# ashvardanian/StringZilla

Hardware: AMD Instinct MI355X
Metric: DP cell-updates/s (GCUPS) on 1M-pair Levenshtein batch (higher is better)
Workload: dtype u32 bit-vectors (u64 results)

## Files before the change

stringzilla_amd/csrc/hip/lev_myers.hip:

```cpp
#include "myers_core.hpp"

#define SZS_PAIR_RULE_FN __host__ __device__ static inline
#include "pair_rule.h"

#include <cstdlib>

namespace szs_hip {

#ifndef SZS_MYERS_PACK_QUERIES
#define SZS_MYERS_PACK_QUERIES 1
#endif
#ifndef SZS_MYERS_PAIR_RULES
#define SZS_MYERS_PAIR_RULES 1
#endif

#ifndef SZS_MYERS_SHORT_TEXT_DWORDS
#define SZS_MYERS_SHORT_TEXT_DWORDS 2
#endif


__device__ __forceinline__ u32 bits_in_word(u32 from, u32 to, int w) {
    u32 const low = from > 32u * w ? from : 32u * w, high = to < 32u * w + 32u ? to : 32u * w + 32u;
    if (low >= high) return 0u;
    return (high - low == 32u ? ~0u : (1u << (high - low)) - 1u) << (low - 32u * w);
}

template <int words_, int text_dwords_, bool runes_, bool paired_ = false>
__device__ __forceinline__ void myers_workgroup(u32 *peq, u32 *keys, szs_string_ref_t const query,
                                                szs_string_ref_t const *__restrict__ candidates, u32 candidates_count,
                                                u32 candidate_block, u64 *__restrict__ results, u64 results_row_stride,
                                                int symmetric, szs_ref_guard_t const &guard, u32 alphabet = 0,
                                                u32 *claimed_rows = nullptr, u32 blocks_here = 1, szs_string_ref_t const second = {}) {
    static_assert(!paired_ || !runes_, "query pairs are a byte-kernel shape");
    constexpr int rows = runes_ ? rune_slots_k : byte_rows_k;
    using layout = peq_layout<words_, rows>;
    if (guard.enabled && (!ref_is_current(guard, 0, query) || (paired_ && !ref_is_current(guard, 0, second)))) {
        if (threadIdx.x == 0) *guard.stale = guard.sequence;
        return;
    }
    u32 const first_length = query.length, second_length = paired_ ? second.length : 0u;
    u32 const query_length = paired_ ? first_length + second_length : first_length;
    u32 const used_rows = paired_ ? query_length + 2u : query_length;
    u32 const pad = 32u * words_ - used_rows;
    u32 const second_row = pad + first_length + 2u;

    for (int i = threadIdx.x; i < layout::total_dwords; i += 256) peq[i] = 0;
    if constexpr (runes_) {
        if (alphabet) {
            for (u32 i = threadIdx.x; i <= alphabet; i += 256) keys[i] = 0;
            if (threadIdx.x == 0) *claimed_rows = 0;
        }
        else
            for (int i = threadIdx.x; i < rune_slots_k; i += 256) keys[i] = rune_slot_empty_k;
    }
    __syncthreads();
    if (runes_ && alphabet) {
        u32 const *pattern = reinterpret_cast<u32 const *>(query.address);
        for (u32 i = threadIdx.x; i < query_length; i += 256) {
            u32 const id = pattern[i];
            if (atomicCAS(&keys[id], 0u, ~0u) == 0u) keys[id] = atomicAdd(claimed_rows, 1u) + 1;
        }
        __syncthreads();
        for (u32 i = threadIdx.x; i < query_length; i += 256) {
            u32 const position = pad + i;
            atomicOr(&peq[layout::dword_index((int)keys[pattern[i]], (int)(position >> 5))], 1u << (position & 31));
        }
    }
    else if constexpr (runes_) {
        u32 const *pattern = reinterpret_cast<u32 const *>(query.address);
        for (u32 i = threadIdx.x; i < query_length; i += 256) {
            u32 const rune = pattern[i];
            u32 slot = rune_slot_hash(rune);
            for (;;) {
                u32 const previous = atomicCAS(&keys[slot], rune_slot_empty_k, rune);
                if (previous == rune_slot_empty_k || previous == rune) break;
                slot = (slot + 1) & (rune_slots_k - 1);
            }
            u32 const position = pad + i;
            atomicOr(&peq[layout::dword_index((int)slot, (int)(position >> 5))], 1u << (position & 31));
        }
    }
    else {
        u8 const *pattern = reinterpret_cast<u8 const *>(query.address);
        for (u32 i = threadIdx.x; i < first_length; i += 256) {
            u32 const position = pad + i;
            atomicOr(&peq[layout::dword_index(pattern[i], (int)(position >> 5))], 1u << (position & 31));
        }
        if constexpr (paired_) {
            u8 const *above = reinterpret_cast<u8 const *>(second.address);
            for (u32 i = threadIdx.x; i < second_length; i += 256) {
                u32 const position = second_row + i;
                atomicOr(&peq[layout::dword_index(above[i], (int)(position >> 5))], 1u << (position & 31));
            }
        }
    }
    __syncthreads();
    pattern_pair_t<words_> boundary;
    if constexpr (paired_) {
#pragma unroll
        for (int w = 0; w < words_; ++w) {
            boundary.separators[w] = bits_in_word(second_row - 2u, second_row, w);
            boundary.tops[w] = first_length ? bits_in_word(second_row - 3u, second_row - 2u, w) : 0u;
        }
    }

#pragma unroll 1
    for (u32 block_step = 0; block_step < blocks_here; ++block_step) {
    u32 const candidate_slot = (candidate_block - block_step) * SZS_CANDIDATES_PER_WORKGROUP + threadIdx.x;
    bool live = candidate_slot < candidates_count;
    szs_string_ref_t candidate = {0, 0, 0};
    if (live) candidate = candidates[candidate_slot];
    if (live && guard.enabled && !ref_is_current(guard, 1, candidate)) {
        *guard.stale = guard.sequence;
        live = false;
    }
    if ((symmetric & SZS_LAYOUT_SYMMETRIC) && candidate.index > query.index) live = false;
    u32 const text_length = live ? candidate.length : 0;
    u32 const longest_in_wave = wave_max_u32(text_length);
    u32 const shortest_in_wave = ~wave_max_u32(live ? ~text_length : 0u);

    u32 vp[words_], vn[words_];
#pragma unroll
    for (int w = 0; w < words_; ++w) {
        vp[w] = bits_in_word(pad, 32u * words_, w) & ~(paired_ ? boundary.separators[w] : 0u);
        vn[w] = 0;
    }

    auto take = [&](u32 symbol) {
        u32 eq[words_];
        load_match_masks<words_, rows>(peq, !runes_ ? symbol : alphabet ? keys[symbol] : find_rune_slot(keys, symbol), eq);
        if constexpr (paired_) myers_column<words_>(vp, vn, eq, boundary);
        else myers_column<words_>(vp, vn, eq);
    };

    u32 column = 0;
    if constexpr (runes_) {
        u32 const *const runes = reinterpret_cast<u32 const *>(candidate.address);
        auto quad_at = [&](u32 index) -> uint4 {
            return index < text_length ? *reinterpret_cast<uint4 const *>(runes + index) : make_uint4(0, 0, 0, 0);
        };
        if (4 <= shortest_in_wave && longest_in_wave) {
            uint4 ahead = quad_at(0);
            for (; column + 4 <= shortest_in_wave; column += 4) {
                uint4 const now = ahead;
                ahead = quad_at(column + 4);
                take(now.x), take(now.y), take(now.z), take(now.w);
            }
        }
#pragma unroll 1
        for (; column < longest_in_wave; ++column)
            if (column < text_length) take(runes[column]);
    }
    else {
        u64 const safe_address = text_length ? candidate.address : first_length || !paired_ ? query.address : second.address;
        text_stream_t text(safe_address, text_length);
        if (!text_length) text.valid_dwords = query_length ? 1 : 0;
        u32 raw_low = text.raw(0);
        u32 dword = 0;
        constexpr u32 columns_per_iteration = 4 * text_dwords_;
#ifndef SZS_MYERS_CLAMPED_READS
#define SZS_MYERS_CLAMPED_READS(TEXT_DWORDS) ((TEXT_DWORDS) == 1)
#endif
        constexpr bool clamped_reads = SZS_MYERS_CLAMPED_READS(text_dwords_);
        if (columns_per_iteration <= shortest_in_wave && longest_in_wave && query_length) {
            u32 ahead[text_dwords_];
#pragma unroll
            for (int d = 0; d < text_dwords_; ++d) ahead[d] = clamped_reads ? text.raw_clamped(1 + d) : text.raw(1 + d);
            for (; column + columns_per_iteration <= shortest_in_wave;
                 column += columns_per_iteration, dword += text_dwords_) {
                u32 symbols[text_dwords_];
                symbols[0] = text.splice(raw_low, ahead[0]);
#pragma unroll
                for (int d = 1; d < text_dwords_; ++d) symbols[d] = text.splice(ahead[d - 1], ahead[d]);
                raw_low = ahead[text_dwords_ - 1];
#pragma unroll
                for (int d = 0; d < text_dwords_; ++d)
                    ahead[d] = clamped_reads ? text.raw_clamped(dword + text_dwords_ + 1 + d)
                                             : text.raw(dword + text_dwords_ + 1 + d);
#pragma unroll
                for (int step = 0; step < 4 * text_dwords_; ++step) take((symbols[step / 4] >> (8 * (step % 4))) & 0xFFu);
            }
        }
#ifndef SZS_MYERS_MID_LOOP
#define SZS_MYERS_MID_LOOP 0
#endif
        if constexpr (SZS_MYERS_MID_LOOP && text_dwords_ > 1) {
            if (column + 4 <= shortest_in_wave && longest_in_wave && query_length) {
                u32 ahead_one = text.raw(dword + 1);
#pragma unroll 1
                for (; column + 4 <= shortest_in_wave; column += 4, ++dword) {
                    u32 const symbols = text.splice(raw_low, ahead_one);
                    raw_low = ahead_one;
                    ahead_one = text.raw(dword + 2);
#pragma unroll
                    for (int step = 0; step < 4; ++step) take((symbols >> (8 * step)) & 0xFFu);
                }
            }
        }
        if (column < longest_in_wave) {
            u32 next = text.raw(dword + 1);
#pragma unroll 1
            for (; column < longest_in_wave; column += 4, ++dword) {
                u32 const after = text.raw(dword + 2);
                u32 const symbols = text.splice(raw_low, next);
                raw_low = next, next = after;
#pragma unroll
                for (int step = 0; step < 4; ++step)
                    if (column + step < text_length) take((symbols >> (8 * step)) & 0xFFu);
            }
        }
    }

    if (live && paired_) {
        u32 first = text_length, above = text_length;
#pragma unroll
        for (int w = 0; w < words_; ++w) {
            u32 const mine = bits_in_word(pad, pad + first_length, w), theirs = bits_in_word(second_row, 32u * words_, w);
            first += (u32)__builtin_popcount(vp[w] & mine) - (u32)__builtin_popcount(vn[w] & mine);
            above += (u32)__builtin_popcount(vp[w] & theirs) - (u32)__builtin_popcount(vn[w] & theirs);
        }
        bool const transposed = (symmetric & SZS_LAYOUT_TRANSPOSED) != 0;
        u64 const one = transposed ? candidate.index : query.index, two = transposed ? candidate.index : second.index;
        u64 const one_column = transposed ? query.index : candidate.index, two_column = transposed ? second.index : candidate.index;
        results[one * results_row_stride + one_column] = first;
        results[two * results_row_stride + two_column] = above;
    }
    else if (live) {
        u32 distance = text_length;
#pragma unroll
        for (int w = 0; w < words_; ++w) distance += (u32)__builtin_popcount(vp[w]) - (u32)__builtin_popcount(vn[w]);
        bool const transposed = (symmetric & SZS_LAYOUT_TRANSPOSED) != 0;
        u64 const row = transposed ? candidate.index : query.index, column = transposed ? query.index : candidate.index;
        results[row * results_row_stride + column] = distance;
        if ((symmetric & SZS_LAYOUT_SYMMETRIC) && candidate.index != query.index)
            results[column * results_row_stride + row] = distance;
    }
    }
}

#ifndef SZS_WORK_BLOCK_MAJOR
#define SZS_WORK_BLOCK_MAJOR 1
#endif
__device__ __forceinline__ void myers_work_item(u32 candidate_blocks, u32 &query_slot, u32 &candidate_block) {
#if SZS_WORK_BLOCK_MAJOR
    u32 const queries_count = gridDim.x / candidate_blocks;
    query_slot = blockIdx.x % queries_count;
    candidate_block = candidate_blocks - 1 - blockIdx.x / queries_count;
#else
    query_slot = blockIdx.x / candidate_blocks;
    candidate_block = candidate_blocks - 1 - blockIdx.x % candidate_blocks;
#endif
}

#ifndef SZS_MYERS_LONG_WAVES
#define SZS_MYERS_LONG_WAVES 2
#endif
template <int words_>
__global__ __launch_bounds__(256, SZS_MYERS_LONG_WAVES) void levenshtein_myers_long_kernel(szs_string_ref_t const *__restrict__ queries,
                                                                      szs_string_ref_t const *__restrict__ candidates,
                                                                      u32 candidates_count, u32 candidate_blocks,
                                                                      u64 *__restrict__ results, u64 results_row_stride,
                                                                      int symmetric, szs_ref_guard_t guard) {
    __shared__ __attribute__((aligned(16))) u32 peq[peq_layout<words_>::total_dwords];
    u32 query_slot, candidate_block;
    myers_work_item(candidate_blocks, query_slot, candidate_block);
    myers_workgroup<words_, 1, false>(peq, nullptr, queries[query_slot], candidates, candidates_count, candidate_block,
                                      results, results_row_stride, symmetric, guard);
}

__device__ __forceinline__ u64 fused_offset(void const *offsets, u32 wide, u64 index) {
    return wide ? static_cast<u64 const *>(offsets)[index] : (u64) static_cast<u32 const *>(offsets)[index];
}

__device__ __forceinline__ void fused_sort_side(szs_plan_side_t const &side, u32 is_query_side, u32 choose_rule, u32 sequence, u32 *ready,
                                                u32 second_ready, u32 withhold, szs_fused_side_report_t *report, u32 *histogram ,
                                                szs_string_ref_t *staged ) {
    constexpr u32 per_thread = SZS_FUSED_MOST_STRINGS / 256;
    u32 const tid = threadIdx.x, lane = tid & 63u, wave = tid >> 6, count = side.count;
    bool const one_pass = count <= SZS_FUSED_MOST_STRINGS;
    __shared__ u32 wave_bins[4], wave_longest[4], wave_status[4];
    __shared__ unsigned long long wave_symbols[4], wave_bands_systolic[4], wave_bands_chain[4], wave_squares[4];
    __shared__ u32 rule_words[256];

    u64 const began = wall_clock64();
    for (u32 bin = tid; bin < SZS_FUSED_BINS; bin += 256) histogram[bin] = 0;
    u64 from[per_thread], to[per_thread];
#pragma unroll
    for (u32 k = 0; k < per_thread; ++k) {
        u32 const i = tid + k * 256;
        from[k] = to[k] = 0;
        if (one_pass && i < count) from[k] = fused_offset(side.offsets, side.wide, i), to[k] = fused_offset(side.offsets, side.wide, (u64)i + 1);
    }
    __syncthreads();
    u32 bins[per_thread];
    u32 status = 0, longest = 0;
    u64 symbols = 0, bands_systolic = 0, bands_chain = 0, squares = 0;
    auto count_in = [&](u64 first, u64 last) -> u32 {
        if (last < first) return status |= SZS_PLAN_STATUS_DESCENDING, ~0u;
        if (last - first > 0xFFFFFFFFull) return status |= SZS_PLAN_STATUS_OVERFLOW, ~0u;
        u32 const length = (u32)(last - first);
        symbols += length, squares += (u64)length * length, longest = length > longest ? length : longest;
        bands_systolic += length ? (length + SZS_SYSTOLIC_BAND_ROWS - 1) / SZS_SYSTOLIC_BAND_ROWS : 1;
        bands_chain += length ? (length + SZS_MYERS_CHAIN_BAND_ROWS - 1) / SZS_MYERS_CHAIN_BAND_ROWS : 1;
        u32 const bin = length < SZS_FUSED_BINS - 1 ? length : SZS_FUSED_BINS - 1;
        atomicAdd(&histogram[bin], 1u);
        return bin;
    };
    if (one_pass) {
#pragma unroll
        for (u32 k = 0; k < per_thread; ++k) {
            bins[k] = ~0u;
            if (tid + k * 256 < count) bins[k] = count_in(from[k], to[k]);
        }
    }
    else {
#pragma unroll 1
        for (u32 first = 0; first < count; first += 1024) {
            u64 some_from[4], some_to[4];
#pragma unroll
            for (u32 k = 0; k < 4; ++k) {
                u32 const i = first + tid + k * 256;
                some_from[k] = some_to[k] = 0;
                if (i < count) some_from[k] = fused_offset(side.offsets, side.wide, i), some_to[k] = fused_offset(side.offsets, side.wide, (u64)i + 1);
            }
#pragma unroll
            for (u32 k = 0; k < 4; ++k)
                if (first + tid + k * 256 < count) (void)count_in(some_from[k], some_to[k]);
        }
    }
    if (tid == 0) report->ticks[0] = (u32)began, report->ticks[1] = (u32)(wall_clock64() - began);
#pragma unroll
    for (int offset = 32; offset >= 1; offset >>= 1) {
        status |= (u32)__shfl_xor((int)status, offset, 64);
        u32 const other = (u32)__shfl_xor((int)longest, offset, 64);
        longest = other > longest ? other : longest;
    }
    if (lane == 0) wave_status[wave] = status, wave_longest[wave] = longest;
    __syncthreads();
    u32 mine[4], sum = 0;
#pragma unroll
    for (u32 k = 0; k < 4; ++k) mine[k] = histogram[4 * tid + k], sum += mine[k];
    u32 inclusive = sum;
#pragma unroll
    for (int offset = 1; offset < 64; offset <<= 1) {
        u32 const other = (u32)__shfl_up((int)inclusive, offset, 64);
        if (lane >= (u32)offset) inclusive += other;
    }
    if (lane == 63) wave_bins[wave] = inclusive;
    __syncthreads();
    status = wave_status[0] | wave_status[1] | wave_status[2] | wave_status[3];
    longest = wave_longest[0];
#pragma unroll
    for (u32 w = 1; w < 4; ++w) longest = wave_longest[w] > longest ? wave_longest[w] : longest;
    u32 running = inclusive - sum;
    for (u32 w = 0; w < wave; ++w) running += wave_bins[w];
#pragma unroll
    for (u32 k = 0; k < 4; ++k) histogram[4 * tid + k] = running, running += mine[k];
    __syncthreads();
    if (tid == 0) report->ticks[2] = (u32)(wall_clock64() - began);
    u32 const blank = status || (is_query_side && longest > 32u * SZS_MYERS_SHORT_WORDS);
    if (one_pass) {
#pragma unroll
        for (u32 k = 0; k < per_thread; ++k) {
            u32 const i = tid + k * 256;
            if (i >= count) continue;
            szs_string_ref_t ref;
            ref.address = status ? side.base : side.base + from[k], ref.length = blank ? 0u : (u32)(to[k] - from[k]), ref.index = i;
            staged[status ? i : atomicAdd(&histogram[bins[k]], 1u)] = ref;
        }
        __syncthreads();
        for (u32 position = tid; position < count; position += 256) {
            szs_string_ref_t const ref = staged[position];
            side.ascending[position] = ref, side.descending[count - 1 - position] = ref;
        }
    }
    u32 const pair_slots = szs_pair_slots(count), pair_seconds = szs_pair_seconds(count);
    bool const choosing = choose_rule && one_pass && pair_seconds;
    if (choosing) {
        constexpr u32 strides = 256 / SZS_PAIR_RULE_CANDIDATES;
        u32 me = tid;
        asm volatile("" : "+v"(me));
        u32 const rule = szs_pair_rule_candidate(me % SZS_PAIR_RULE_CANDIDATES, pair_seconds);
        u32 words = 0;
        if (me < strides * SZS_PAIR_RULE_CANDIDATES) {
#pragma unroll 4
            for (u32 slot = me / SZS_PAIR_RULE_CANDIDATES; slot < pair_seconds; slot += strides)
                words += szs_pair_slot_words(staged[count - 1 - slot].length,
                                             staged[count - 1 - szs_pair_second_rank(rule, slot, pair_slots, pair_seconds)].length);
        }
        rule_words[me] = words;
    }
    if (!one_pass) {
#pragma unroll 1
        for (u32 first = 0; first < count; first += 1024) {
            u64 some_from[4], some_to[4];
#pragma unroll
            for (u32 k = 0; k < 4; ++k) {
                u32 const i = first + tid + k * 256;
                some_from[k] = some_to[k] = 0;
                if (i < count) some_from[k] = fused_offset(side.offsets, side.wide, i), some_to[k] = fused_offset(side.offsets, side.wide, (u64)i + 1);
            }
#pragma unroll
            for (u32 k = 0; k < 4; ++k) {
                u32 const i = first + tid + k * 256;
                if (i >= count) continue;
// ... 1351 lines not shown
```

stringzilla_amd/csrc/hip/myers_core.hpp:

```cpp
#pragma once
#include "device_common.hpp"

namespace szs_hip {

constexpr int byte_rows_k = 256;
constexpr int rune_slots_k = 512;
constexpr u32 rune_slot_empty_k = ~0u;

template <int words_, int rows_ = byte_rows_k>
struct peq_layout {
    static constexpr int chunk_words = words_ >= 3 ? 4 : words_;
    static constexpr int chunks = (words_ + chunk_words - 1) / chunk_words;
    static constexpr int total_dwords = chunks * rows_ * chunk_words;
    __device__ static constexpr int dword_index(int row, int w) {
        return ((w / chunk_words) * rows_ + row) * chunk_words + (w % chunk_words);
    }
};

__device__ __forceinline__ u32 rune_slot_hash(u32 rune) { return (rune * 2654435761u) >> 23; }
__device__ __forceinline__ u32 find_rune_slot(u32 const *keys, u32 rune) {
    u32 slot = rune_slot_hash(rune);
    for (;;) {
        u32 const key = keys[slot];
        if (key == rune || key == rune_slot_empty_k) return slot;
        slot = (slot + 1) & (rune_slots_k - 1);
    }
}

template <int words_, int rows_>
__device__ __forceinline__ void load_match_masks(u32 const *peq, u32 symbol, u32 (&eq)[words_]) {
    using layout = peq_layout<words_, rows_>;
    if constexpr (layout::chunk_words == 4) {
        uint4 const *rows = reinterpret_cast<uint4 const *>(peq);
#pragma unroll
        for (int chunk = 0; chunk < layout::chunks; ++chunk) {
            uint4 const row = rows[chunk * rows_ + symbol];
            if (chunk * 4 + 0 < words_) eq[chunk * 4 + 0] = row.x;
            if (chunk * 4 + 1 < words_) eq[chunk * 4 + 1] = row.y;
            if (chunk * 4 + 2 < words_) eq[chunk * 4 + 2] = row.z;
            if (chunk * 4 + 3 < words_) eq[chunk * 4 + 3] = row.w;
        }
    }
    else if constexpr (layout::chunk_words == 2) {
        uint2 const row = reinterpret_cast<uint2 const *>(peq)[symbol];
        eq[0] = row.x, eq[1] = row.y;
    }
    else { eq[0] = peq[symbol]; }
}

__device__ __forceinline__ bool ref_is_current(szs_ref_guard_t const &guard, int side, szs_string_ref_t const &ref) {
    if (ref.index >= guard.side[side].count) return false;
    u64 from, to;
    if (guard.side[side].wide) {
        u64 const *offsets = static_cast<u64 const *>(guard.side[side].offsets);
        from = offsets[ref.index], to = offsets[(u64)ref.index + 1];
    }
    else {
        u32 const *offsets = static_cast<u32 const *>(guard.side[side].offsets);
        from = offsets[ref.index], to = offsets[(u64)ref.index + 1];
    }
    return to >= from && to - from == ref.length && guard.side[side].base + from == ref.address;
}

struct single_pattern_t {
    __device__ static constexpr u32 separator(int) { return 0; }
    __device__ static constexpr u32 top(int) { return 0; }
};

template <int words_>
struct pattern_pair_t {
    u32 separators[words_], tops[words_];
    __device__ u32 separator(int w) const { return separators[w]; }
    __device__ u32 top(int w) const { return tops[w]; }
};

template <int words_, typename boundary_t = single_pattern_t, bool materialise_ = true>
__device__ __forceinline__ void myers_column(u32 (&vp)[words_], u32 (&vn)[words_], u32 const (&eq)[words_],
                                             boundary_t const &boundary = {}) {
    u32 carry = 0, hp_below = 0, hn_below = 0;
#pragma unroll
    for (int w = 0; w < words_; ++w) {
        u32 xv = eq[w] | vn[w];
        if constexpr (!std::is_same<boundary_t, single_pattern_t>::value)
            asm("v_bitop3_b32 %0, %1, %2, %3 bitop3:0xfe" : "=v"(xv) : "v"(eq[w]), "v"(vn[w]), "v"(boundary.separator(w)));
        u32 carry_out;
        u32 const sum = __builtin_addc(eq[w] & vp[w], vp[w], carry, &carry_out);
        carry = carry_out;
        u32 const d0 = (sum ^ vp[w]) | eq[w];
        u32 const hp = vn[w] | ~(d0 | vp[w]);
        u32 const hn = vp[w] & d0 & ~boundary.top(w);
        u32 const hp_shifted = w == 0 ? ((hp << 1) | 1u) : __builtin_amdgcn_alignbit(hp, hp_below, 31);
        u32 const hn_shifted = w == 0 ? (hn << 1) : __builtin_amdgcn_alignbit(hn, hn_below, 31);
        hp_below = hp, hn_below = hn;
        vp[w] = hn_shifted | ~(xv | hp_shifted);
        vn[w] = hp_shifted & xv & ~boundary.separator(w);
        if constexpr (materialise_ && words_ > 1) asm("" : "+v"(vp[w]), "+v"(vn[w]));
    }
}

template <int words_>
__device__ __forceinline__ u32 myers_infix_column(u32 (&vp)[words_], u32 (&vn)[words_], u32 const (&eq)[words_]) {
    u32 carry = 0, hp_below = 0, hn_below = 0;
#pragma unroll
    for (int w = 0; w < words_; ++w) {
        u32 const xv = eq[w] | vn[w];
        u32 carry_out;
        u32 const sum = __builtin_addc(eq[w] & vp[w], vp[w], carry, &carry_out);
        carry = carry_out;
        u32 const d0 = (sum ^ vp[w]) | eq[w];
        u32 const hp = vn[w] | ~(d0 | vp[w]);
        u32 const hn = vp[w] & d0;
        u32 const hp_shifted = w == 0 ? (hp << 1) : __builtin_amdgcn_alignbit(hp, hp_below, 31);
        u32 const hn_shifted = w == 0 ? (hn << 1) : __builtin_amdgcn_alignbit(hn, hn_below, 31);
        hp_below = hp, hn_below = hn;
        vp[w] = hn_shifted | ~(xv | hp_shifted);
        vn[w] = hp_shifted & xv;
        if constexpr (words_ > 1) asm("" : "+v"(vp[w]), "+v"(vn[w]));
    }
    return (hp_below >> 31) | ((hn_below >> 31) << 1);
}

template <int words_>
__device__ __forceinline__ u32 myers_prefix_column(u32 (&vp)[words_], u32 (&vn)[words_], u32 const (&eq)[words_]) {
    u32 carry = 0, hp_below = 0, hn_below = 0;
#pragma unroll
    for (int w = 0; w < words_; ++w) {
        u32 const xv = eq[w] | vn[w];
        u32 carry_out;
        u32 const sum = __builtin_addc(eq[w] & vp[w], vp[w], carry, &carry_out);
        carry = carry_out;
        u32 const d0 = (sum ^ vp[w]) | eq[w];
        u32 const hp = vn[w] | ~(d0 | vp[w]);
        u32 const hn = vp[w] & d0;
        u32 const hp_shifted = w == 0 ? ((hp << 1) | 1u) : __builtin_amdgcn_alignbit(hp, hp_below, 31);
        u32 const hn_shifted = w == 0 ? (hn << 1) : __builtin_amdgcn_alignbit(hn, hn_below, 31);
        hp_below = hp, hn_below = hn;
        vp[w] = hn_shifted | ~(xv | hp_shifted);
        vn[w] = hp_shifted & xv;
        if constexpr (words_ > 1) asm("" : "+v"(vp[w]), "+v"(vn[w]));
    }
    return (hp_below >> 31) | ((hn_below >> 31) << 1);
}

template <int words_>
__device__ __forceinline__ u32 myers_strip_column(u32 (&vp)[words_], u32 (&vn)[words_], u32 const (&eq)[words_], u32 hp_in,
                                                  u32 hn_in) {
    u32 carry = 0, hp_below = 0, hn_below = 0;
#pragma unroll
    for (int w = 0; w < words_; ++w) {
        u32 const xv = eq[w] | vn[w];
        u32 const eq_in = w == 0 ? (eq[w] | hn_in) : eq[w];
        u32 carry_out;
        u32 const sum = __builtin_addc(eq_in & vp[w], vp[w], carry, &carry_out);
        carry = carry_out;
        u32 const d0 = (sum ^ vp[w]) | eq_in;
        u32 const hp = vn[w] | ~(d0 | vp[w]);
        u32 const hn = vp[w] & d0;
        u32 const hp_shifted = w == 0 ? ((hp << 1) | hp_in) : __builtin_amdgcn_alignbit(hp, hp_below, 31);
        u32 const hn_shifted = w == 0 ? ((hn << 1) | hn_in) : __builtin_amdgcn_alignbit(hn, hn_below, 31);
        hp_below = hp, hn_below = hn;
        vp[w] = hn_shifted | ~(xv | hp_shifted);
        vn[w] = hp_shifted & xv;
    }
    return (hp_below >> 31) | ((hn_below >> 31) << 1);
}

}
```

stringzilla_amd/csrc/hip/myers_rerank.hip:

```cpp
#include "rerank_core.hpp"

namespace szs_hip {

template <int words_, int lanes_>
__device__ __forceinline__ void rerank_rows(u32 *table, listed_row_t const &row, szs_rerank_side_t const &candidates,
                                            u64 const *__restrict__ indices, u64 indices_stride, u64 k, u64 *__restrict__ scores,
                                            u64 scores_stride, u32 *flags, unsigned long long *counters) {
    u32 const sub = threadIdx.x % lanes_;
    u32 const pad = 32u * words_ - row.query_length;
    listed_table<words_, lanes_>(table, row, [](int) { return 0u; }, [&](u32 i) { return pad + i; });

    listed_counters_t counted;
#pragma unroll 1
    for (u64 first = 0; first < k; first += lanes_) {
        u64 const rank = first + sub;
        u64 const at = row.row * scores_stride + rank;
        u64 address = 0;
        u32 text_length = 0;
        bool const live = row.has_row && rank < k &&
                          listed_candidate(candidates, indices[row.row * indices_stride + rank], [&]() { scores[at] = 0; }, flags, address, text_length);

        u32 vp[words_], vn[words_];
#pragma unroll
        for (int w = 0; w < words_; ++w) vp[w] = rerank_bits_in_word(pad, 32u * words_, w), vn[w] = 0;
        listed_walk(
            text_stream_t(address, text_length), text_length, live,
            [&](u32 symbol, u32) {
                u32 eq[words_];
                load_match_masks<words_, byte_rows_k>(table, symbol, eq);
                myers_column<words_>(vp, vn, eq);
            },
            []() { return true; });

        if (live) {
            u32 distance = text_length;
#pragma unroll
            for (int w = 0; w < words_; ++w) distance += (u32)__builtin_popcount(vp[w]) - (u32)__builtin_popcount(vn[w]);
            scores[at] = distance;
            counted.add(row.query_length, text_length);
        }
    }
    counted.land(counters, true);
}

template <int lanes_>
__global__ __launch_bounds__(64) void levenshtein_rerank_kernel(szs_rerank_side_t const queries, szs_rerank_side_t const candidates,
                                                                u64 const first_query, u32 const *__restrict__ rows, u32 const rows_count,
                                                                u64 const *__restrict__ indices, u64 const indices_stride, u64 const k,
                                                                u64 *__restrict__ scores, u64 const scores_stride, u32 const table_dwords,
                                                                u32 *flags, unsigned long long *counters) {
    extern __shared__ __attribute__((aligned(16))) u32 rerank_tables[];
    listed_one_strip_rows<lanes_>(queries, first_query, rows, rows_count, rerank_tables, table_dwords, flags,
                                  [&](auto width, u32 *table, listed_row_t const &row) {
                                      rerank_rows<decltype(width)::value, lanes_>(table, row, candidates, indices, indices_stride, k, scores,
                                                                                  scores_stride, flags, counters);
                                  });
}

}

extern "C" unsigned szs_hip_rerank_lanes(uint64_t k) { return k <= 16 ? 16u : k <= 32 ? 32u : 64u; }

extern "C" int szs_hip_levenshtein_rerank(szs_rerank_side_t const *queries, szs_rerank_side_t const *candidates, uint64_t first_query,
                                          uint32_t const *rows, uint32_t rows_count, uint64_t const *indices, uint64_t indices_stride,
                                          uint64_t k, uint64_t *scores, uint64_t scores_stride, unsigned widest, uint32_t *flags,
                                          unsigned long long *counters, void *stream) {
    using namespace szs_hip;
    if (!rows_count || !k) return 0;
    if (widest < 1 || widest > SZS_MYERS_SHORT_WORDS || !queries || !candidates || !flags || !counters) return (int)hipErrorInvalidValue;
    listed_grid_t const grid = listed_one_strip_grid(k, rows_count, widest);
    return listed_launch(k, [&](auto lanes) {
        hipLaunchKernelGGL(levenshtein_rerank_kernel<decltype(lanes)::value>, dim3(grid.grid), dim3(wave_size_k), grid.lds,
                           static_cast<hipStream_t>(stream), *queries, *candidates, first_query, rows, rows_count, indices, indices_stride, k,
                           scores, scores_stride, grid.table_dwords, flags, counters);
    });
}
```

Before: 101,800.

## Rederive Myers column via shifted HN carry identity and bitop3 ternary ops

Rewrites the Myers bit-vector column update so the shifted horizontal-negative vector comes straight from the add's carry bits (sum ^ (eq|vp) ^ eq), removing the separate HN shift chain, and fuses most boolean steps into v_bitop3_b32 ternary instructions. For query pairs the boundary handling moves from a per-column 'top' mask to a 'lower' mask folded into the kept term, and the separator row is pre-seeded in the PEQ table at initialisation. This aims to cut VALU instructions and carried registers per DP column, in exchange for hand-derived truth tables that must stay exactly correct for paired boundaries. The rerank path opts out of spelled carries so the compiler can pick its own form.

Result: faster. 119,500, median of 6 (+17.4%).

```diff
diff --git a/stringzilla_amd/csrc/hip/lev_myers.hip b/stringzilla_amd/csrc/hip/lev_myers.hip
--- a/stringzilla_amd/csrc/hip/lev_myers.hip
+++ b/stringzilla_amd/csrc/hip/lev_myers.hip
@@ -44,7 +44,13 @@
     u32 const pad = 32u * words_ - used_rows;
     u32 const second_row = pad + first_length + 2u;
 
-    for (int i = threadIdx.x; i < layout::total_dwords; i += 256) peq[i] = 0;
+    if constexpr (paired_) {
+        u32 const s0_dword = (second_row - 2u) >> 5, s0_mask = 1u << ((second_row - 2u) & 31u);
+        for (int i = threadIdx.x; i < layout::total_dwords; i += 256)
+            peq[i] = (u32)(i / (rows * layout::chunk_words) * layout::chunk_words + i % layout::chunk_words) == s0_dword ? s0_mask : 0u;
+    }
+    else
+        for (int i = threadIdx.x; i < layout::total_dwords; i += 256) peq[i] = 0;
     if constexpr (runes_) {
         if (alphabet) {
             for (u32 i = threadIdx.x; i <= alphabet; i += 256) keys[i] = 0;
@@ -100,7 +106,7 @@
 #pragma unroll
         for (int w = 0; w < words_; ++w) {
             boundary.separators[w] = bits_in_word(second_row - 2u, second_row, w);
-            boundary.tops[w] = first_length ? bits_in_word(second_row - 3u, second_row - 2u, w) : 0u;
+            boundary.lower[w] = bits_in_word(second_row - 2u, second_row - 1u, w);
         }
     }
 
diff --git a/stringzilla_amd/csrc/hip/myers_core.hpp b/stringzilla_amd/csrc/hip/myers_core.hpp
--- a/stringzilla_amd/csrc/hip/myers_core.hpp
+++ b/stringzilla_amd/csrc/hip/myers_core.hpp
@@ -62,38 +62,47 @@
     return to >= from && to - from == ref.length && guard.side[side].base + from == ref.address;
 }
 
-struct single_pattern_t {
-    __device__ static constexpr u32 separator(int) { return 0; }
-    __device__ static constexpr u32 top(int) { return 0; }
-};
+struct single_pattern_t {};
 
 template <int words_>
 struct pattern_pair_t {
-    u32 separators[words_], tops[words_];
-    __device__ u32 separator(int w) const { return separators[w]; }
-    __device__ u32 top(int w) const { return tops[w]; }
+    u32 separators[words_], lower[words_];
 };
 
-template <int words_, typename boundary_t = single_pattern_t, bool materialise_ = true>
+template <int table_>
+__device__ __forceinline__ u32 bitop3(u32 a, u32 b, u32 c) {
+    u32 r;
+    asm("v_bitop3_b32 %0, %1, %2, %3 bitop3:%4" : "=v"(r) : "v"(a), "v"(b), "v"(c), "n"(table_));
+    return r;
+}
+
+template <int words_, typename boundary_t = single_pattern_t, bool materialise_ = true, bool spelled_carries_ = true>
 __device__ __forceinline__ void myers_column(u32 (&vp)[words_], u32 (&vn)[words_], u32 const (&eq)[words_],
                                              boundary_t const &boundary = {}) {
-    u32 carry = 0, hp_below = 0, hn_below = 0;
+    constexpr bool paired = !std::is_same<boundary_t, single_pattern_t>::value;
+    static_assert(spelled_carries_ || !paired, "a pair's HNs is not a function the compiler finds by itself");
+    u32 carry = 0, hp_below = 0;
 #pragma unroll
     for (int w = 0; w < words_; ++w) {
-        u32 xv = eq[w] | vn[w];
-        if constexpr (!std::is_same<boundary_t, single_pattern_t>::value)
-            asm("v_bitop3_b32 %0, %1, %2, %3 bitop3:0xfe" : "=v"(xv) : "v"(eq[w]), "v"(vn[w]), "v"(boundary.separator(w)));
+        u32 xv, kept, hn_shifted;
+        if constexpr (paired) {
+            xv = bitop3<0xfe>(eq[w], vn[w], boundary.separators[w]);
+            kept = bitop3<0x54>(eq[w], vp[w], boundary.lower[w]);
+        }
+        else
+            xv = eq[w] | vn[w], kept = eq[w] | vp[w];
         u32 carry_out;
         u32 const sum = __builtin_addc(eq[w] & vp[w], vp[w], carry, &carry_out);
         carry = carry_out;
-        u32 const d0 = (sum ^ vp[w]) | eq[w];
-        u32 const hp = vn[w] | ~(d0 | vp[w]);
-        u32 const hn = vp[w] & d0 & ~boundary.top(w);
+        if constexpr (paired) hn_shifted = bitop3<0x94>(sum, kept, eq[w]);
+        else if constexpr (spelled_carries_) hn_shifted = bitop3<0x96>(sum, kept, eq[w]);
+        else hn_shifted = sum ^ kept ^ eq[w];
+        u32 const hp = bitop3<0xf1>(vn[w], sum, kept);
         u32 const hp_shifted = w == 0 ? ((hp << 1) | 1u) : __builtin_amdgcn_alignbit(hp, hp_below, 31);
-        u32 const hn_shifted = w == 0 ? (hn << 1) : __builtin_amdgcn_alignbit(hn, hn_below, 31);
-        hp_below = hp, hn_below = hn;
-        vp[w] = hn_shifted | ~(xv | hp_shifted);
-        vn[w] = hp_shifted & xv & ~boundary.separator(w);
+        hp_below = hp;
+        vp[w] = bitop3<0xf1>(hn_shifted, xv, hp_shifted);
+        if constexpr (paired) vn[w] = bitop3<0x40>(hp_shifted, xv, boundary.separators[w]);
+        else vn[w] = hp_shifted & xv;
         if constexpr (materialise_ && words_ > 1) asm("" : "+v"(vp[w]), "+v"(vn[w]));
     }
 }
diff --git a/stringzilla_amd/csrc/hip/myers_rerank.hip b/stringzilla_amd/csrc/hip/myers_rerank.hip
--- a/stringzilla_amd/csrc/hip/myers_rerank.hip
+++ b/stringzilla_amd/csrc/hip/myers_rerank.hip
@@ -28,7 +28,7 @@
             [&](u32 symbol, u32) {
                 u32 eq[words_];
                 load_match_masks<words_, byte_rows_k>(table, symbol, eq);
-                myers_column<words_>(vp, vn, eq);
+                myers_column<words_, single_pattern_t, true, false>(vp, vn, eq);
             },
             []() { return true; });
 
```
